# ZhentaoHuang/SealD-NeRF

Hardware: AMD Instinct MI355X
Metric: rendered rays/sec + sampled-points/sec, 800×800 D-NeRF jumpingjacks (higher is better)
Workload: dtype f16; 1 GPU; dnerf jumpingjacks-like 800x800 full-frame inference render, -O (fp16 field network, fp16 grid table), test sequence of 20 frames (camera orbit, one time stamp per frame, t = 0 .. 1: every frame selects its own occupancy slice, time encoding and the t == 0 canonical rule), T_thresh 1e-2, max_steps 1024, dt_gamma 0; rays=640000, field=fused, loop=device, frames_per_loop=4, rays_per_loop_on_this_gpu=2560000, frames_in_flight=4 loops of 4 frame(s) (the next starts when the newest is down to rays/2 alive), parallelism=single GPU

## Files before the change

### include/sdn_hip.h

```cpp
#ifndef SDN_HIP_H
#define SDN_HIP_H

#include <stdint.h>

#ifdef __cplusplus
extern "C" {
#endif

#define SDN_F32 0
#define SDN_F16 1

#define SDN_E_BADARG (-1)
#define SDN_E_UNSUPPORTED (-2)
#define SDN_E_TIMEOUT (-3)

const char *sdn_version(void);
int sdn_debug_shader_clock(unsigned long long *out4, uint32_t wall_ticks, void *stream);


int sdn_near_far_from_aabb(const float *rays_o, const float *rays_d, const float *aabb, uint32_t N,
                           float min_near, float *nears, float *fars, void *stream);

int sdn_sph_from_ray(const float *rays_o, const float *rays_d, float radius, uint32_t N, float *coords,
                     void *stream);
// ... 98 lines not shown

uint32_t sdn_field_basis_weight_floats_f32(void);
int sdn_field_basis_forward_f32(const float *xyzs, const float *dirs, const uint32_t *live_idx, const uint32_t *live_count,
                                uint32_t M, const float *weights, const float *basis_row , const float *table,
                                const int32_t *offsets_host, float S, uint32_t H, float bound, float density_scale,
                                float *sigmas, float *rgbs, void *stream);

uint32_t sdn_field_hyper_weight_blocks(void);
int sdn_field_hyper_forward_f16(const float *xyzs, const float *dirs, const uint32_t *live_idx, const uint32_t *live_count,
                                uint32_t M, const void *weights, const float *ambient_row , const void *table,
                                const int32_t *offsets_host, float S, uint32_t H, float bound, float density_scale,
                                float *sigmas, float *rgbs, void *stream);

void sdn_field_select_kernel(int persistent);
void sdn_field_persistent_workgroups(int n);

int sdn_field_build_quad_table(const void *embeddings, int dtype, const int32_t *ref_offsets_host, float S, uint32_t H, void *out,
                               void *stream);
int sdn_field_build_quad_table_nd(const void *embeddings, int dtype, uint32_t input_dim, const int32_t *ref_offsets_host, float S,
                                  uint32_t H, void *out, void *stream);

int sdn_density_query_cells_f16(const int32_t *cells, const uint32_t *cell_count, uint32_t n, const float *noise, uint32_t seed,
                                uint32_t grid_size, float cas_bound, const void *weights, const float *bias0, const void *table,
                                const int32_t *offsets_host, float S, uint32_t H, float bound, float density_scale, int zero_deform,
                                float *tmp_slice, void *stream);
int sdn_density_query_cells_f32(const int32_t *cells, const uint32_t *cell_count, uint32_t n, const float *noise, uint32_t seed,
                                uint32_t grid_size, float cas_bound, const float *weights, const float *bias0, const float *table,
                                const int32_t *offsets_host, float S, uint32_t H, float bound, float density_scale, int zero_deform,
                                float *tmp_slice, void *stream);
int sdn_density_query_cells_basis_f16(const int32_t *cells, const uint32_t *cell_count, uint32_t n, const float *noise, uint32_t seed,
// ... 110 lines not shown
    float *xyzs, *dirs, *deltas, *sigmas, *rgbs;
    uint32_t *live_idx;
    int32_t *live_counts, *state, *trace, *n_out;
    void *block_totals;
    const void *field_weights;
    const float *field_bias0;
    const void *grid_table;
    int32_t grid_offsets[17];
    float grid_S;
    uint32_t grid_H;
    uint32_t N, M_cap, n_counters, max_steps, C, H;
    float bound, dt_gamma, T_thresh, density_scale;
    int32_t zero_deform;
    const float *aabb;
    float min_near;
    int32_t reserved_;
    float *rays_tend;
    const struct SdnSealBox *seal;
    uint8_t *seal_mask;
    uint32_t n_group_frames, rays_per_frame;
    const uint8_t *frame_bitfield[SDN_MAX_GROUP_FRAMES];
    uint8_t *slot_frame;
    const void *frame_cull[SDN_MAX_GROUP_FRAMES];
    int32_t field_f32;
    int32_t reserved2_;
    const float *noises;
    const struct SdnSealBrush *seal_brush;
} SdnRenderCtx;

int sdn_render_begin(const SdnRenderCtx *ctx, void *stream);
int sdn_render_step_f16(const SdnRenderCtx *ctx, uint32_t bound_alive, void *stream);
int sdn_render_step_f16_ev(const SdnRenderCtx *ctx, uint32_t bound_alive, void *ev_field_begin, void *ev_field_end,
                           void *stream);
int sdn_render_time_kernel(int which);
int sdn_render_frame_f16(const SdnRenderCtx *ctx, float bg_color, float *image_out, float *depth_out, void *stream,
                         void *side_stream, void **ev_main, void **ev_copy, int32_t *host_snap, void **ev_field,
                         uint32_t max_field_events, uint32_t *iterations_out);
int sdn_render_frames_pipelined_f16(const SdnRenderCtx *const *ctxs, uint32_t n_ctx, uint32_t n_frames, const float *const *rays_o,
                                    const float *const *rays_d, float *const *image_outs, float *const *depth_outs, float bg_color,
                                    uint32_t overlap_div, void *const *streams, void *const *side_streams, void **ev_main,
// ... 133 lines not shown
```

### seald-nerf_amd/csrc/field.hip

```cpp
#include <math.h>
#include <type_traits>
#include <stdlib.h>

#include "sdn_common.h"
#include "sdn_internal.h"
#include "cell_points.h"
#include "grid_common.h"
#include "field_f16_net.h"

namespace {

using namespace sdn_f16;

#ifdef SDN_STAMPS
constexpr uint32_t kStampWGs = 2048;
__device__ unsigned long long g_field_stamps[kStampWGs * 2 * 32];
#define FSTAMP(k) do { __builtin_amdgcn_sched_barrier(0); if (stamp_on) { stamp_slot[k] = __builtin_amdgcn_s_memtime(); } __builtin_amdgcn_sched_barrier(0); } while (0)
#else
#define FSTAMP(k) ((void)0)
#endif

constexpr int kStageBytes = 32768;
constexpr int kWaves = 8;
constexpr int kPointsPerWG = 32 * kWaves;
// ... 270 lines not shown
    auto row = [&](uint32_t rr) {
        const T *p = emb + (size_t)(a + rr % hs) * 2;
        const __half2 v = __halves2half2(__float2half_rn((float)p[0]), __float2half_rn((float)p[1]));
        return __builtin_bit_cast(uint32_t, v);
    };
    out[i + 2u * l] = make_uint4(row(r), row(r + 1u), row(r + s1), row(r + s1 + 1u));
}

}

namespace sdn_int {

static int g_field_pp = -1;
static int g_field_pp_wgs = 0;
constexpr uint32_t kPPMinTilesPerCU = 4;

int field_table_layout(const int32_t *offsets_host) { return table_layout(offsets_host); }
int fill_tiled_levels_nd(TiledLevels &lv, uint32_t (*s3)[16], uint32_t D, const int32_t *offsets_host, float S, uint32_t H) {
    return fill_tiled_levels(lv, offsets_host, S, H, D, s3 ? *s3 : nullptr);
}
int fill_field_args(FieldArgs &a, TiledLevels &lv, const FieldCall &f) {
    int rc = fill_tiled_levels(lv, f.offsets_host, f.S, f.H);
    if (rc) return rc;
    fill_field_record(a, f);
    return 0;
}
void fill_field_record(FieldArgs &a, const FieldCall &f) {
    a.xyzs = f.xyzs; a.dirs = f.dirs; a.live_idx = f.live_idx; a.live_count = f.live_count; a.state = f.state; a.M = f.M;
    a.weights = (const unsigned char *)f.weights; a.bias0 = f.bias0; a.table = (const __half *)f.table;
    a.sigmas = f.sigmas; a.rgbs = f.rgbs; a.bound = f.bound; a.density_scale = f.density_scale; a.zero_deform = f.zero_deform;
// ... 28 lines not shown
    bool small = busy <= (uint32_t)cus;
    {
        static int pin = -1;
        if (pin < 0) {
            const char *e = getenv("SDN_FIELD_VARIANT");
            pin = !e ? 0 : (e[0] == 't' ? 1 : (e[0] == 'l' ? 2 : 0));
        }
        if (pin == 1) small = false;
        if (pin == 2) small = true;
    }
    const int layout = table_layout(f.offsets_host);
    if (g_field_pp < 0) {
        const char *e = getenv("SDN_FIELD_PP");
        g_field_pp = e ? atoi(e) : 1;
    }
    if (g_field_pp && layout == kLayoutQuad && busy >= kPPMinTilesPerCU * (uint32_t)cus && a.n_frames <= kPPMaxFrames && M < (1u << 28)) {
        const uint32_t pairs = sdn_div_up(M, kPPTile);
        int pp_cus = g_field_pp_wgs > 0 ? g_field_pp_wgs : cus;
        if (pp_cus > cus) pp_cus = cus;
        static int balance = -1;
        if (balance < 0) {
            const char *e = getenv("SDN_FIELD_PP_BALANCE");
            balance = e ? atoi(e) : 0;
        }
        const uint32_t grid = balance == 1 ? (uint32_t)cus : (uint32_t)pp_cus;
        a.pp_soft = (uint32_t)pp_cus | (balance == 0 ? 0x80000000u : (balance == 2 ? 0x40000000u : 0u));
        hipLaunchKernelGGL(k_field_pp_f16, dim3(pairs < grid ? pairs : grid), dim3(64 * kPPWaves), 0, st, a, lv);
        return sdn_launch_status();
    }
    launch_tile<false>(layout, small, wgs, a, lv, st);
    return sdn_launch_status();
}

int field_cells_f16(const FieldCells &q, hipStream_t st) {
    TiledLevels lv;
    FieldArgs a;
    int rc = fill_field_args(a, lv, q.f);
    if (rc) return rc;
    a.cell_noise = q.noise; a.cell_seed = q.seed;
    const float half_grid = q.cas_bound / (float)q.grid_size;
    a.cell_inv = 1.0f / (float)(q.grid_size - 1); a.cell_span = q.cas_bound - half_grid; a.cell_half = half_grid;
    const uint32_t wgs = sdn_div_up(q.f.M, (uint32_t)kPointsPerWG);
    const int layout = table_layout(q.f.offsets_host);
    if (layout == kLayoutRef) return SDN_E_UNSUPPORTED;
    launch_tile<true>(layout, wgs <= 256u, wgs, a, lv, st);
    return sdn_launch_status();
}

}

extern "C" {

uint32_t sdn_field_weight_blocks(void) { return (uint32_t)kBlkTotal; }

void sdn_field_select_kernel(int persistent) { sdn_int::g_field_pp = persistent; }
void sdn_field_persistent_workgroups(int n) { sdn_int::g_field_pp_wgs = n > 0 ? n : 0; }

int sdn_field_build_quad_table(const void *embeddings, int dtype, const int32_t *ref_offsets_host, float S, uint32_t H, void *out, void *stream) {
    return sdn_field_build_quad_table_nd(embeddings, dtype, 3, ref_offsets_host, S, H, out, stream);
}
int sdn_field_build_quad_table_nd(const void *embeddings, int dtype, uint32_t input_dim, const int32_t *ref_offsets_host, float S, uint32_t H, void *out,
                                  void *stream) {
    if (!embeddings || !ref_offsets_host || !out || ((uintptr_t)out & 15u) != 0) return SDN_E_BADARG;
    TiledLevels lv;
    uint32_t s3[16];
    int rc = fill_tiled_levels(lv, ref_offsets_host, S, H, input_dim, s3);
    if (rc) return rc;
    QuadLevels q;
    for (int l = 0; l < 17; l++) q.src[l] = (uint32_t)ref_offsets_host[l];
    for (int l = 0; l < 16; l++) q.s1[l] = lv.s1[l];
    const uint32_t rows = q.src[16];
// ... 19 lines not shown
}
uint32_t sdn_debug_field_stamp_words(void) { return kStampWGs * 2 * 32; }
int sdn_debug_field_stamps(unsigned long long *out) {
    if (!out) return SDN_E_BADARG;
    if (hipDeviceSynchronize() != hipSuccess) return sdn_launch_status();
    if (hipMemcpyFromSymbol(out, HIP_SYMBOL(g_field_stamps), sizeof(unsigned long long) * kStampWGs * 2 * 32) != hipSuccess) return sdn_launch_status();
    void *p = nullptr;
    if (hipGetSymbolAddress(&p, HIP_SYMBOL(g_field_stamps)) != hipSuccess) return sdn_launch_status();
    return (int)hipMemset(p, 0, sizeof(unsigned long long) * kStampWGs * 2 * 32);
}
#endif

int sdn_field_forward_f16(const float *xyzs, const float *dirs, const uint32_t *live_idx, const uint32_t *live_count, uint32_t M,
                          const void *weights, const float *bias0, const void *table, const int32_t *offsets_host, float S, uint32_t H,
                          float bound, float density_scale, int zero_deform, float *sigmas, float *rgbs, void *stream) {
    return sdn_int::field_forward_checked(0, {.xyzs = xyzs, .dirs = dirs, .live_idx = live_idx, .live_count = live_count, .M = M, .weights = weights,
                                              .bias0 = bias0, .table = table, .offsets_host = offsets_host, .S = S, .H = H, .bound = bound,
                                              .density_scale = density_scale, .zero_deform = zero_deform ? 1 : 0, .sigmas = sigmas, .rgbs = rgbs},
                                          stream);
}

}
```

### seald-nerf_amd/csrc/render.hip

```cpp
#include <atomic>
#include <chrono>
#include <stdio.h>
#include <stdlib.h>
#include <string.h>

#include "sdn_common.h"
#include "sdn_internal.h"

namespace sdn_int {
int render_begin(const SdnRenderCtx *c, void *mailbox, uint32_t frame_tag, hipStream_t st) {
    if (c->aabb) {
        int rc0 = sdn_near_far_from_aabb(c->rays_o, c->rays_d, c->aabb, c->N, c->min_near, (float *)c->nears, (float *)c->fars, st);
        if (rc0) return rc0;
    }
    int rc = loop_begin(*c, mailbox, frame_tag, st);
    if (rc) return rc;
    if (has_loop_cull(*c)) {
        const uint32_t nf = c->n_group_frames > 1 ? c->n_group_frames : 1u;
        bool kept = true;
        for (uint32_t f = 0; f < nf; f++) kept = kept && c->frame_cull[f] != nullptr;
        if (kept) rc = copy_cull(c->frame_cull, nf, (uint32_t *)c->cull_bits, st);
        else rc = c->n_group_frames > 1 ? build_cull_group(frame_sel(*c), (uint32_t *)c->cull_bits, st) : build_cull(c->bitfield, (uint32_t *)c->cull_bits, st);
        if (!rc && c->rays_tend) rc = loop_cull_start(*c, st);
    }
// ... 45 lines not shown
    int rc = 0;
    if (s->modify_hsv) rc = sdn_seal_modify_hsv(c.rgbs, c.seal_mask, m_slots, s->hsv[0], s->hsv[1], s->hsv[2], st);
    if (!rc && s->modify_rgb) {
        if (!s->scratch) return SDN_E_BADARG;
        rc = sdn_seal_modify_rgb(c.rgbs, c.seal_mask, m_slots, s->rgb[0], s->rgb[1], s->rgb[2], s->rgb_light_offset, s->scratch, c.live_idx,
                                 sdn_int::live_counters(c), c.state, st);
    }
    if (!rc && s->kind == SDN_SEAL_BRUSH && c.seal_brush && c.seal_brush->image) {
        if (!s->scratch) return SDN_E_BADARG;
        rc = sdn_seal_modify_image(c.rgbs, c.xyzs, c.seal_mask, m_slots, c.seal_brush->image, (char *)s->scratch + 32, c.live_idx,
                                   sdn_int::live_counters(c), c.state, st);
    }
    return rc;
}

static int launch_field(const SdnRenderCtx &c, uint32_t m_bound, uint32_t expect_points, hipStream_t st) {
    const bool group = c.n_group_frames > 1;
    return sdn_int::field_forward(c.field_f32,
                                  {.xyzs = c.xyzs, .dirs = c.dirs, .live_idx = c.live_idx, .live_count = sdn_int::live_counters(c), .state = c.state,
                                   .M = m_bound, .weights = c.field_weights, .bias0 = c.field_bias0, .table = c.grid_table,
                                   .offsets_host = c.grid_offsets, .S = c.grid_S, .H = c.grid_H, .bound = c.bound,
                                   .density_scale = c.density_scale, .zero_deform = c.zero_deform, .sigmas = c.sigmas, .rgbs = c.rgbs,
                                   .expect_points = expect_points, .slot_frame = group ? c.slot_frame : nullptr,
                                   .n_frames = group ? c.n_group_frames : 1u},
                                  st);
}

static uint32_t slot_bound(const SdnRenderCtx &c, uint32_t bound_alive) {
    const uint64_t m = (uint64_t)bound_alive * 8u;
    return m > c.N ? c.N : (uint32_t)m;
}
struct IterEvents { void *field0, *field1, *march0, *march1; };
static IterEvents split_events(void *e0, void *e1) {
    return g_timed_kernel.load() == 1 ? IterEvents{nullptr, nullptr, e0, e1} : IterEvents{e0, e1, nullptr, nullptr};
}
static void record(void *ev, hipStream_t st) { if (ev) (void)hipEventRecord((hipEvent_t)ev, st); }
static int map_field_color(const SdnRenderCtx &c, uint32_t m_slots, uint32_t expect_points, const IterEvents &ev, hipStream_t st) {
    int rc = seal_map(c, m_slots, st);
    if (rc) return rc;
    record(ev.field0, st);
    rc = launch_field(c, m_slots, expect_points, st);
    record(ev.field1, st);
    return rc ? rc : seal_color(c, m_slots, st);
}

static bool stepwise_noises_unsupported(const SdnRenderCtx *c) { return c->noises && c->n_group_frames > 1; }

static bool ctx_ok(const SdnRenderCtx *c) {
    if (!(c && c->rays_o && c->rays_d && c->nears && c->fars && c->alive_a && c->alive_b && c->rays_t && c->weights_sum &&
          c->depth && c->image && c->state && c->live_counts && c->cull_bits))
        return false;
    if (c->n_group_frames > 1) {
        if (c->n_group_frames > SDN_MAX_GROUP_FRAMES || !c->slot_frame || c->rays_per_frame == 0 ||
            (uint64_t)c->n_group_frames * c->rays_per_frame != c->N)
            return false;
        for (uint32_t f = 0; f < c->n_group_frames; f++)
// ... 1 lines not shown
        return true;
    }
    return c->bitfield != nullptr;
}

int sdn_render_begin(const SdnRenderCtx *c, void *stream) {
    if (!ctx_ok(c)) return SDN_E_BADARG;
    if (stepwise_noises_unsupported(c)) return SDN_E_UNSUPPORTED;
    return sdn_int::render_begin(c, nullptr, 0, (hipStream_t)stream);
}

int sdn_render_step_f16(const SdnRenderCtx *c, uint32_t bound_alive, void *stream) {
    return sdn_render_step_f16_ev(c, bound_alive, nullptr, nullptr, stream);
}

int sdn_render_step_f16_ev(const SdnRenderCtx *c, uint32_t bound_alive, void *ev_field_begin, void *ev_field_end, void *stream) {
    if (!c || bound_alive == 0) return SDN_E_BADARG;
    if (bound_alive > c->N) bound_alive = c->N;
    hipStream_t st = (hipStream_t)stream;
    const IterEvents ev = split_events(ev_field_begin, ev_field_end);
    record(ev.march0, st);
    int rc = sdn_int::loop_march(*c, bound_alive, st);
    record(ev.march1, st);
    if (!rc) rc = map_field_color(*c, slot_bound(*c, bound_alive), 0u, ev, st);
    return rc ? rc : sdn_int::loop_composite_compact(*c, bound_alive, st);
}

}

namespace {

constexpr uint32_t kRecompactMin = 8192;
uint32_t recompact_pct(uint32_t list_len) { return list_len > 81920u ? 95u : 50u; }
constexpr int kDriverTimeoutSeconds = 20;

struct FrameRun {
    const SdnRenderCtx *c;
    hipStream_t st, side;
    void **ev_main, **ev_copy, **ev_field;
    int32_t *host_snap;
    uint32_t max_field_events;
    uint32_t bound, it;
    bool steady, done;
    bool recompact = false;
    uint32_t list_bound = 0;
    void *mail_dev = nullptr;
    uint32_t tag = 0;
    uint32_t last_alive = 0;

    int begin() {
        if (!ctx_ok(c)) return SDN_E_BADARG;
        bound = c->N; it = 0; steady = false; done = false; last_alive = c->N; recompact = false; list_bound = 0;
        mail_dev = nullptr;
        unsigned int flags = 0;
        void *dptr = nullptr;
        if (hipHostGetFlags(&flags, host_snap) == hipSuccess && (flags & hipHostMallocCoherent) &&
            hipHostGetDevicePointer(&dptr, host_snap, 0) == hipSuccess && dptr) {
            static std::atomic<uint32_t> frame_seq{0};
            tag = (frame_seq.fetch_add(1) % 0x7FFFu) + 1u;
            mail_dev = dptr;
        } else {
            (void)hipGetLastError();
        }
        return sdn_int::render_begin(c, mail_dev, tag, st);
    }

    int enqueue() {
        void *e0 = (ev_field && it < max_field_events) ? ev_field[2 * it] : nullptr;
        void *e1 = (ev_field && it < max_field_events) ? ev_field[2 * it + 1] : nullptr;
        int rc;
        if (!steady) {
            rc = sdn_render_step_f16_ev(c, bound, e0, e1, st);
        } else {
            const IterEvents ev = split_events(e0, e1);
            rc = map_field_color(*c, slot_bound(*c, bound), last_alive * 8u, ev, st);
            if (!rc) record(ev.march0, st);
            if (!rc && recompact) {
                rc = sdn_int::loop_composite_compact(*c, bound, st, true);
                const uint32_t nb = last_alive < bound ? last_alive : bound;
                if (!rc) rc = sdn_int::loop_steady_begin(*c, nb, st, true);
                bound = list_bound = nb;
                recompact = false;
            } else if (!rc)
                rc = sdn_int::loop_composite_march(*c, bound, st);
            if (!rc) record(ev.march1, st);
        }
        if (rc) return rc;
        if (mail_dev) return 0;
        const uint32_t slot = it & 3u;
        hipError_t e = hipEventRecord((hipEvent_t)ev_main[slot], st);
// ... 108 lines not shown
        if (frame_times) {
            const SdnFrameTime &ft = frame_times[next];
            if (!ft.field_bias0 || !ft.bitfield[0]) return SDN_E_BADARG;
            local[slot].bitfield = ft.bitfield[0];
            for (uint32_t f = 0; f < SDN_MAX_GROUP_FRAMES; f++) local[slot].frame_bitfield[f] = ft.bitfield[f];
            for (uint32_t f = 0; f < SDN_MAX_GROUP_FRAMES; f++) local[slot].frame_cull[f] = ft.cull_grid[f];
            local[slot].field_bias0 = ft.field_bias0;
            local[slot].zero_deform = (int32_t)ft.zero_deform;
        }
        void **evf = ev_field_frames ? (void **)ev_field_frames[next] : nullptr;
        runs[slot] = FrameRun{&local[slot], (hipStream_t)streams[slot], (hipStream_t)side_streams[slot], ev_main + 4 * slot, ev_copy + 4 * slot,
                              evf, host_snap + 8 * slot, evf ? max_field_events : 0u, 0, 0, false, false};
        frame_of[slot] = (int)next++;
        return runs[slot].begin();
    };
    const bool stats = getenv("SDN_DRIVER_STATS") != nullptr;
    double t_work = 0, t_idle = 0;
    uint32_t n_loops = 0;
    auto now = [] { return std::chrono::duration<double, std::micro>(std::chrono::steady_clock::now().time_since_epoch()).count(); };
    auto launch_next = [&]() -> int {
        if (next >= n_frames) return 0;
        const uint32_t slot = next % n_ctx;
        if (frame_of[slot] >= 0) return 0;
        int newest = -1;
        bool any_active = false, excl_in_flight = false;
        for (uint32_t c = 0; c < n_ctx; c++) {
            if (frame_of[c] < 0) continue;
            any_active = true;
            if (newest < 0 || frame_of[c] > frame_of[newest]) newest = (int)c;
            if (exclusive_frames && exclusive_frames[frame_of[c]]) excl_in_flight = true;
        }
        bool ok = !any_active || (uint64_t)runs[newest].last_alive * overlap_div <= local[slot].N;
        if (exclusive_frames && any_active && (exclusive_frames[next] || excl_in_flight)) ok = false;
        if (!ok) return 0;
        int r = start(slot);
        if (!r) r = runs[slot].enqueue();
        return r;
    };
    auto fail = [&](int code) -> int {
        for (uint32_t c = 0; c < n_ctx; c++) { (void)hipStreamSynchronize((hipStream_t)streams[c]); (void)hipStreamSynchronize((hipStream_t)side_streams[c]); }
        (void)hipGetLastError();
        return code;
    };
    int rc = launch_next();
    if (rc) return fail(rc);
    auto t_last = stats ? now() : 0.0;
    uint32_t idle_spins = 0;
    auto t_progress = std::chrono::steady_clock::now();
    auto t_query = t_progress;
    while (finished < n_frames) {
        n_loops++;
// ... 9 lines not shown
            progress = true;
            rc = runs[s2].settle();
            if (rc) return fail(rc);
            if (runs[s2].done) {
                const int f = frame_of[s2];
                rc = sdn_render_finish(&local[s2], bg_color, image_outs[f], depth_outs[f], streams[s2]);
                if (rc) return fail(rc);
                if (done_events && done_events[f]) {
                    hipError_t e = hipEventRecord((hipEvent_t)done_events[f], (hipStream_t)streams[s2]);
                    if (e != hipSuccess) return fail((int)e);
                }
                if (iterations_out) __atomic_store_n(&iterations_out[f], runs[s2].it + 1, __ATOMIC_RELEASE);
                frame_of[s2] = -1;
                finished++;
            } else {
                rc = runs[s2].enqueue();
                if (rc) return fail(rc);
            }
            rc = launch_next();
            if (rc) return fail(rc);
        }
        if (!progress) {
            rc = launch_next();
            if (rc) return fail(rc);
            if ((++idle_spins & 0x3FFFu) == 0) {
                const auto now_c = std::chrono::steady_clock::now();
                if (now_c - t_progress > std::chrono::milliseconds(5) && now_c - t_query > std::chrono::milliseconds(5)) {
                    t_query = now_c;
                    for (uint32_t c = 0; c < n_ctx; c++)
                        if (frame_of[c] >= 0) { hipError_t q = hipStreamQuery((hipStream_t)streams[c]); if (q != hipSuccess && q != hipErrorNotReady) return fail((int)q); }
// ... 34 lines not shown
```

### seald-nerf_amd/csrc/sdn_internal.h

```cpp
#pragma once
#include "sdn_common.h"

namespace sdn_int {

struct FrameSel {
    uint32_t n_frames = 0;
    uint32_t rays_per_frame = 0;
    uint32_t cull_stride = 0;
    uint32_t pad_ = 0;
    const uint8_t *grid[SDN_MAX_GROUP_FRAMES] = {};
    uint8_t *slot_frame = nullptr;
};
FrameSel frame_sel(const SdnRenderCtx &c);

inline int32_t *snap_ring(const SdnRenderCtx &c) { return c.trace + 2 * (size_t)c.n_counters; }
inline int32_t *snap_n_out(const SdnRenderCtx &c) { return snap_ring(c) + 8; }
inline uint32_t *live_counters(const SdnRenderCtx &c) { return (uint32_t *)c.live_counts; }
inline float *jump_buffer(const SdnRenderCtx &c) { return c.rays_tend ? c.sigmas : nullptr; }
inline bool has_loop_cull(const SdnRenderCtx &c) { return c.H == 128 && c.C == 1; }
inline const uint32_t *loop_cull(const SdnRenderCtx &c) { return has_loop_cull(c) ? (const uint32_t *)c.cull_bits : nullptr; }

int loop_begin(const SdnRenderCtx &c, void *mailbox, uint32_t frame_tag, hipStream_t st);
int loop_cull_start(const SdnRenderCtx &c, hipStream_t st);
int loop_march(const SdnRenderCtx &c, uint32_t bound_alive, hipStream_t st);
// ... 15 lines not shown
    const int32_t *state = nullptr;
    uint32_t M = 0;
    const void *weights = nullptr;
    const float *bias0 = nullptr;
    const void *table = nullptr;
    const int32_t *offsets_host = nullptr;
    float S = 0;
    uint32_t H = 0;
    float bound = 0, density_scale = 0;
    int zero_deform = 0;
    float *sigmas = nullptr, *rgbs = nullptr;
    float *deform = nullptr;
    uint32_t expect_points = 0;
    const uint8_t *slot_frame = nullptr;
    uint32_t n_frames = 1;
};
struct FieldCells {
    FieldCall f;
    const float *noise = nullptr;
    uint32_t seed = 0, grid_size = 0;
    float cas_bound = 0;
};

inline uint32_t field_n_frames(const FieldCall &f) {
    if (!f.slot_frame || f.n_frames == 0) return 1u;
    return f.n_frames > (uint32_t)SDN_MAX_GROUP_FRAMES ? (uint32_t)SDN_MAX_GROUP_FRAMES : f.n_frames;
}

int field_forward_f16(const FieldCall &f, hipStream_t st);
int field_forward_f32(const FieldCall &f, hipStream_t st);
// ... 52 lines not shown
```

### seald-nerf_amd/dnerf_amd/frame_loops.py

```python
import ctypes
import os
import sys
from time import perf_counter
from types import SimpleNamespace

import numpy as np
import torch

import raymarching
import sdn_backend
from sdn_backend import lib, check, ptr, stream
from .dist import InOrderHandOn


def sample_capacity(N):
    return N + 128 + 8 * 128


def flat_rays(rays):
    return rays.contiguous().view(-1, 3)


def per_frame_times(time, n, mismatch, spread_single=False):
    times = list(time) if isinstance(time, (list, tuple)) else [time] * n
# ... 373 lines not shown
                raise RuntimeError(f"hipStreamCreateWithPriority failed ({rc})")
            out.append(torch.cuda.ExternalStream(h.value, device=device))
    _CONTEXT_STREAMS[key] = out
    return out


_CONTEXT_STREAMS = {}


class PipelinedDeviceLoop:

    def __init__(self, model, field, N, device, overlap_div=1, contexts=2, mailbox=True, **kw):
        self.N, self.device, self.overlap_div, self.K = N, device, int(overlap_div), int(contexts)
        self.loops = [DeviceLoop(model, field, N, device, mailbox=mailbox, **kw) for _ in range(self.K)]
        self.streams = _context_streams(self.K, device)
        if self.K > 1:
            lib.sdn_field_persistent_workgroups(int(torch.cuda.get_device_properties(device).multi_processor_count) * 7 // 8)
        self.host_state = sdn_backend.HostMailbox(self.K) if mailbox else torch.zeros(self.K, 8, dtype=torch.int32).pin_memory()
        self._ctxs = (ctypes.POINTER(sdn_backend.SdnRenderCtx) * self.K)(*[ctypes.pointer(lp.ctx) for lp in self.loops])
        self._fixed = None

    @torch.no_grad()
    def render_frames(self, rays_o, rays_d, time, bg_color=1.0, outputs=None, timing=None, exclusive=None, on_done=None, perturb=False,
                      noises=None):
        t_entry = perf_counter()
        if perturb or noises is not None:
            raise NotImplementedError("a perturbed first march is not built for pipelined frames: render preview frames with DeviceLoop")
        n = len(rays_o)
        assert n == len(rays_d) and n >= 1
        cur = torch.cuda.current_stream()
        ro = [flat_rays(r) for r in rays_o]
        rd = [flat_rays(r) for r in rays_d]
# ... 161 lines not shown
```

### seald-nerf_amd/sdn_backend.py

```python
import ctypes
import os
import weakref

import torch

_HERE = os.path.dirname(os.path.abspath(__file__))
LIB_PATH = os.environ.get("SDN_LIB_PATH") or os.path.join(_HERE, "lib", "libsdn_hip.so")

SDN_F32 = 0
SDN_F16 = 1

_c = ctypes
_vp, _u32, _f32, _i32, _u64 = _c.c_void_p, _c.c_uint32, _c.c_float, _c.c_int, _c.c_uint64

PROTOTYPES = {
    "sdn_near_far_from_aabb": [_vp, _vp, _vp, _u32, _f32, _vp, _vp, _vp],
    "sdn_sph_from_ray": [_vp, _vp, _f32, _u32, _vp, _vp],
    "sdn_get_rays": [_vp, _f32, _f32, _f32, _f32, _u32, _u32, _vp, _vp, _vp],
    "sdn_morton3D": [_vp, _u32, _vp, _vp],
    "sdn_morton3D_invert": [_vp, _u32, _vp, _vp],
    "sdn_packbits": [_vp, _u32, _f32, _vp, _vp],
    "sdn_march_rays_train": [_vp, _vp, _vp, _f32, _f32, _u32, _u32, _u32, _u32, _u32, _vp, _vp, _vp, _vp, _vp, _vp, _vp, _vp, _vp, _vp],
    "sdn_composite_rays_train_forward": [_vp, _vp, _vp, _vp, _u32, _u32, _f32, _vp, _vp, _vp, _vp],
    "sdn_composite_whole_rays": [_vp, _vp, _vp, _vp, _vp, _u32, _u32, _f32, _vp, _vp, _vp, _vp],
# ... 20 lines not shown
    "sdn_render_frame_f16": [_vp, _f32, _vp, _vp, _vp, _vp, _vp, _vp, _vp, _vp, _u32, _vp],
    "sdn_render_frames_pipelined_f16": [_vp, _u32, _u32, _vp, _vp, _vp, _vp, _f32, _u32, _vp, _vp, _vp, _vp, _vp, _vp, _u32, _vp, _vp, _vp, _vp],
    "sdn_host_mailbox_free": [_vp],
    "sdn_seal_bbox_map": [_vp, _vp, _u32, _vp, _u32, _vp, _u32, _vp, _vp, _vp, _vp, _vp, _vp, _vp],
    "sdn_seal_modify_hsv": [_vp, _vp, _u32, _f32, _f32, _f32, _vp],
    "sdn_seal_bbox_map_source": [_vp, _vp, _u32, _vp, _u32, _vp, _u32, _vp, _vp, _vp, _vp, _vp, _vp, _vp, _vp, _vp, _vp, _vp, _vp, _vp],
    "sdn_seal_anchor_map": [_vp, _vp, _u32, _vp, _u32, _vp, _u32, _vp, _vp, _vp, _vp, _f32, _f32, _vp, _vp, _vp, _vp, _vp, _vp, _vp],
    "sdn_seal_brush_map": [_vp, _vp, _u32, _vp, _u32, _vp, _u32, _vp, _vp, _vp, _f32, _u32, _vp, _u32, _vp, _vp],
    "sdn_seal_modify_rgb": [_vp, _vp, _u32, _f32, _f32, _f32, _f32, _vp, _vp, _vp, _vp, _vp],
    "sdn_whole_rays_schedule": [_vp, _vp, _vp, _u32, _u32, _f32, _u32, _vp, _vp, _vp, _vp],
    "sdn_seal_modify_rgb_whole_rays": [_vp, _vp, _vp, _vp, _vp, _u32, _u32, _f32, _u32, _f32, _f32, _f32, _f32, _vp, _vp, _vp, _vp, _vp],
    "sdn_seal_image_texels": [_vp, _u64, _vp],
    "sdn_seal_modify_image": [_vp, _vp, _vp, _u32, _vp, _vp, _vp, _vp, _vp, _vp],
    "sdn_seal_modify_image_whole_rays": [_vp, _vp, _vp, _vp, _vp, _vp, _u32, _u32, _f32, _u32, _vp, _vp, _vp, _vp, _vp, _vp],
    "sdn_field_forward_f16": [_vp, _vp, _vp, _vp, _u32, _vp, _vp, _vp, _vp, _f32, _u32, _f32, _f32, _i32, _vp, _vp, _vp],
    "sdn_field_forward_f32": [_vp, _vp, _vp, _vp, _u32, _vp, _vp, _vp, _vp, _f32, _u32, _f32, _f32, _i32, _vp, _vp, _vp, _vp],
    "sdn_field_forward_f32x3": [_vp, _vp, _vp, _vp, _u32, _vp, _vp, _vp, _vp, _f32, _u32, _f32, _f32, _i32, _vp, _vp, _vp, _vp],
    "sdn_field_basis_forward_f16": [_vp, _vp, _vp, _vp, _u32, _vp, _vp, _vp, _vp, _f32, _u32, _f32, _f32, _vp, _vp, _vp],
    "sdn_field_basis_forward_f32": [_vp, _vp, _vp, _vp, _u32, _vp, _vp, _vp, _vp, _f32, _u32, _f32, _f32, _vp, _vp, _vp],
    "sdn_density_query_cells_basis_f32": [_vp, _vp, _u32, _vp, _u32, _u32, _f32, _vp, _vp, _vp, _vp, _f32, _u32, _f32, _f32, _vp, _vp],
    "sdn_field_hyper_forward_f16": [_vp, _vp, _vp, _vp, _u32, _vp, _vp, _vp, _vp, _f32, _u32, _f32, _f32, _vp, _vp, _vp],
    "sdn_field_build_quad_table": [_vp, _i32, _vp, _f32, _u32, _vp, _vp],
    "sdn_field_build_quad_table_nd": [_vp, _i32, _u32, _vp, _f32, _u32, _vp, _vp],
    "sdn_grid_encode_forward_quad_f16": [_vp, _vp, _vp, _vp, _u32, _f32, _u32, _vp],
    "sdn_density_query_cells_f16": [_vp, _vp, _u32, _vp, _u32, _u32, _f32, _vp, _vp, _vp, _vp, _f32, _u32, _f32, _f32, _i32, _vp, _vp],
    "sdn_debug_shader_clock": [_vp, _u32, _vp],
    "sdn_density_query_cells_f32": [_vp, _vp, _u32, _vp, _u32, _u32, _f32, _vp, _vp, _vp, _vp, _f32, _u32, _f32, _f32, _i32, _vp, _vp],
    "sdn_density_query_cells_basis_f16": [_vp, _vp, _u32, _vp, _u32, _u32, _f32, _vp, _vp, _vp, _vp, _f32, _u32, _f32, _f32, _vp, _vp],
    "sdn_density_query_cells_hyper_f16": [_vp, _vp, _u32, _vp, _u32, _u32, _f32, _vp, _vp, _vp, _vp, _f32, _u32, _f32, _f32, _vp, _vp],
    "sdn_density_grid_ema": [_vp, _vp, ctypes.c_uint64, _f32, _vp, _vp],
# ... 9 lines not shown


class SdnFrameTime(ctypes.Structure):
    _fields_ = [("bitfield", _vp * MAX_GROUP_FRAMES), ("field_bias0", _vp), ("zero_deform", _u32), ("reserved_", _u32),
                ("cull_grid", _vp * MAX_GROUP_FRAMES)]


class SdnRenderCtx(ctypes.Structure):
    _fields_ = ([(n, _vp) for n in ("rays_o", "rays_d", "nears", "fars", "bitfield", "cull_bits", "alive_a", "alive_b", "rays_t",
                                   "weights_sum", "depth", "image", "xyzs", "dirs", "deltas", "sigmas", "rgbs", "live_idx",
                                   "live_counts", "state", "trace", "n_out", "block_totals", "field_weights", "field_bias0",
                                   "grid_table")]
                + [("grid_offsets", ctypes.c_int32 * 17), ("grid_S", _f32), ("grid_H", _u32)]
                + [(n, _u32) for n in ("N", "M_cap", "n_counters", "max_steps", "C", "H")]
                + [(n, _f32) for n in ("bound", "dt_gamma", "T_thresh", "density_scale")]
                + [("zero_deform", ctypes.c_int32), ("aabb", _vp), ("min_near", _f32), ("reserved_", ctypes.c_int32), ("rays_tend", _vp), ("seal", _vp), ("seal_mask", _vp),
                   ("n_group_frames", _u32), ("rays_per_frame", _u32), ("frame_bitfield", _vp * MAX_GROUP_FRAMES), ("slot_frame", _vp),
                   ("frame_cull", _vp * MAX_GROUP_FRAMES), ("field_f32", _i32), ("reserved2_", _i32), ("noises", _vp), ("seal_brush", _vp)])


LOOP_WORDS = ("n_alive", "n_step", "steps_done", "iteration", "side", "N", "max_steps", "advance_calls", "frozen_len", "survivors",
              "mailbox_lo", "mailbox_hi", "frame_tag", "tend_lo", "tend_hi", "culled_start")
(LOOP_N_ALIVE, LOOP_N_STEP, LOOP_STEPS_DONE, LOOP_ITERATION, LOOP_SIDE, LOOP_N, LOOP_MAX_STEPS, LOOP_ADVANCE_CALLS, LOOP_FROZEN_LEN,
 LOOP_SURVIVORS, LOOP_MAILBOX_LO, LOOP_MAILBOX_HI, LOOP_FRAME_TAG, LOOP_TEND_LO, LOOP_TEND_HI, LOOP_CULLED_START) = range(len(LOOP_WORDS))


class SdnSealBox(ctypes.Structure):
    _fields_ = [("bounds", _f32 * 24), ("n_bounds", _u32), ("n_tris", _u32), ("tris", _vp), ("test_dir", _f32 * 3), ("tinv", _f32 * 12),
                ("rinv", _f32 * 9), ("scale", _f32 * 3), ("center", _f32 * 3), ("hsv", _f32 * 3), ("modify_hsv", ctypes.c_int32),
                ("rgb", _f32 * 3), ("rgb_light_offset", _f32), ("modify_rgb", ctypes.c_int32), ("has_map_source", ctypes.c_int32),
                ("source_bound", _f32 * 6), ("map_source", _f32 * 3), ("reserved_", _u32), ("scratch", _vp), ("kind", _u32),
                ("v_anchor", _f32 * 3), ("v_offset", _f32 * 3), ("v_h", _f32 * 3), ("len_h", _f32), ("radius", _f32)]

# ... 265 lines not shown
```

Before: 3.220 billion sampled-points/s.

## Pick persistent field kernel workgroup share per loop from in-flight concurrency

Replaces the global 7/8-of-CUs persistent-workgroup cap, set once in Python when several contexts exist, with a per-loop share computed by the pipelined driver. A loop running alone with no loops waiting gets all CUs with balanced dealing. Otherwise it gets 7/8 of the CUs with exact dealing. The aim is to let tail loops use the whole GPU while keeping headroom for overlapping loops in steady state, at the cost of extra host logic per enqueue and possible contention changes.

```diff
diff --git a/include/sdn_hip.h b/include/sdn_hip.h
--- a/include/sdn_hip.h
+++ b/include/sdn_hip.h
@@ -136,6 +136,12 @@
 
 void sdn_field_select_kernel(int persistent);
 void sdn_field_persistent_workgroups(int n);
+int sdn_field_forward_f16_share(const float *xyzs, const float *dirs, const uint32_t *live_idx, const uint32_t *live_count,
+                                uint32_t M, const void *weights, const float *bias0, const void *table,
+                                const int32_t *offsets_host, float S, uint32_t H, float bound, float density_scale,
+                                int zero_deform, float *sigmas, float *rgbs, uint32_t pp_workgroups, uint32_t pp_deal,
+                                void *stream);
+int sdn_field_persistent_last_launch(uint32_t *out);
 
 int sdn_field_build_quad_table(const void *embeddings, int dtype, const int32_t *ref_offsets_host, float S, uint32_t H, void *out,
                                void *stream);
@@ -276,7 +282,7 @@
     int32_t zero_deform;
     const float *aabb;
     float min_near;
-    int32_t reserved_;
+    uint32_t pp_workgroups;
     float *rays_tend;
     const struct SdnSealBox *seal;
     uint8_t *seal_mask;
@@ -285,7 +291,7 @@
     uint8_t *slot_frame;
     const void *frame_cull[SDN_MAX_GROUP_FRAMES];
     int32_t field_f32;
-    int32_t reserved2_;
+    uint32_t pp_deal;
     const float *noises;
     const struct SdnSealBrush *seal_brush;
 } SdnRenderCtx;
diff --git a/seald-nerf_amd/csrc/field.hip b/seald-nerf_amd/csrc/field.hip
--- a/seald-nerf_amd/csrc/field.hip
+++ b/seald-nerf_amd/csrc/field.hip
@@ -1,4 +1,5 @@
 #include <math.h>
+#include <atomic>
 #include <type_traits>
 #include <stdlib.h>
 
@@ -308,6 +309,7 @@
 static int g_field_pp = -1;
 static int g_field_pp_wgs = 0;
 constexpr uint32_t kPPMinTilesPerCU = 4;
+static std::atomic<uint32_t> g_pp_launches{0}, g_pp_last_wgs{0}, g_pp_last_deal{0}, g_pp_last_grid{0};
 
 int field_table_layout(const int32_t *offsets_host) { return table_layout(offsets_host); }
 int fill_tiled_levels_nd(TiledLevels &lv, uint32_t (*s3)[16], uint32_t D, const int32_t *offsets_host, float S, uint32_t H) {
@@ -366,18 +368,22 @@
         const char *e = getenv("SDN_FIELD_PP");
         g_field_pp = e ? atoi(e) : 1;
     }
-    if (g_field_pp && layout == kLayoutQuad && busy >= kPPMinTilesPerCU * (uint32_t)cus && a.n_frames <= kPPMaxFrames && M < (1u << 28)) {
+    const uint32_t pp_min_tiles = g_field_pp > 1 ? (uint32_t)g_field_pp : kPPMinTilesPerCU * (uint32_t)cus;
+    if (g_field_pp && layout == kLayoutQuad && busy >= pp_min_tiles && a.n_frames <= kPPMaxFrames && M < (1u << 28)) {
         const uint32_t pairs = sdn_div_up(M, kPPTile);
-        int pp_cus = g_field_pp_wgs > 0 ? g_field_pp_wgs : cus;
-        if (pp_cus > cus) pp_cus = cus;
-        static int balance = -1;
-        if (balance < 0) {
+        const uint32_t pp_cus = f.pp_workgroups > 0 && f.pp_workgroups < (uint32_t)cus ? f.pp_workgroups : (uint32_t)cus;
+        static int balance_env = -2;
+        if (balance_env == -2) {
             const char *e = getenv("SDN_FIELD_PP_BALANCE");
-            balance = e ? atoi(e) : 0;
-        }
-        const uint32_t grid = balance == 1 ? (uint32_t)cus : (uint32_t)pp_cus;
-        a.pp_soft = (uint32_t)pp_cus | (balance == 0 ? 0x80000000u : (balance == 2 ? 0x40000000u : 0u));
-        hipLaunchKernelGGL(k_field_pp_f16, dim3(pairs < grid ? pairs : grid), dim3(64 * kPPWaves), 0, st, a, lv);
+            balance_env = e ? atoi(e) : -1;
+        }
+        const uint32_t balance = balance_env >= 0 ? (uint32_t)balance_env : f.pp_deal;
+        const uint32_t grid_cus = balance == kPPDealBalanced ? (uint32_t)cus : pp_cus;
+        const uint32_t grid = pairs < grid_cus ? pairs : grid_cus;
+        a.pp_soft = pp_cus | (balance == kPPDealExact ? 0x80000000u : (balance == kPPDealCapped ? 0x40000000u : 0u));
+        g_pp_last_wgs = pp_cus; g_pp_last_deal = balance; g_pp_last_grid = grid;
+        g_pp_launches++;
+        hipLaunchKernelGGL(k_field_pp_f16, dim3(grid), dim3(64 * kPPWaves), 0, st, a, lv);
         return sdn_launch_status();
     }
     launch_tile<false>(layout, small, wgs, a, lv, st);
@@ -407,6 +413,11 @@
 
 void sdn_field_select_kernel(int persistent) { sdn_int::g_field_pp = persistent; }
 void sdn_field_persistent_workgroups(int n) { sdn_int::g_field_pp_wgs = n > 0 ? n : 0; }
+int sdn_field_persistent_last_launch(uint32_t *out) {
+    if (!out) return SDN_E_BADARG;
+    out[0] = sdn_int::g_pp_launches; out[1] = sdn_int::g_pp_last_wgs; out[2] = sdn_int::g_pp_last_deal; out[3] = sdn_int::g_pp_last_grid;
+    return 0;
+}
 
 int sdn_field_build_quad_table(const void *embeddings, int dtype, const int32_t *ref_offsets_host, float S, uint32_t H, void *out, void *stream) {
     return sdn_field_build_quad_table_nd(embeddings, dtype, 3, ref_offsets_host, S, H, out, stream);
@@ -456,9 +467,18 @@
 int sdn_field_forward_f16(const float *xyzs, const float *dirs, const uint32_t *live_idx, const uint32_t *live_count, uint32_t M,
                           const void *weights, const float *bias0, const void *table, const int32_t *offsets_host, float S, uint32_t H,
                           float bound, float density_scale, int zero_deform, float *sigmas, float *rgbs, void *stream) {
+    return sdn_field_forward_f16_share(xyzs, dirs, live_idx, live_count, M, weights, bias0, table, offsets_host, S, H, bound, density_scale, zero_deform,
+                                       sigmas, rgbs, (uint32_t)sdn_int::g_field_pp_wgs, sdn_int::kPPDealExact, stream);
+}
+int sdn_field_forward_f16_share(const float *xyzs, const float *dirs, const uint32_t *live_idx, const uint32_t *live_count, uint32_t M,
+                                const void *weights, const float *bias0, const void *table, const int32_t *offsets_host, float S, uint32_t H,
+                                float bound, float density_scale, int zero_deform, float *sigmas, float *rgbs, uint32_t pp_workgroups,
+                                uint32_t pp_deal, void *stream) {
+    if (pp_deal > sdn_int::kPPDealCapped) return SDN_E_BADARG;
     return sdn_int::field_forward_checked(0, {.xyzs = xyzs, .dirs = dirs, .live_idx = live_idx, .live_count = live_count, .M = M, .weights = weights,
                                               .bias0 = bias0, .table = table, .offsets_host = offsets_host, .S = S, .H = H, .bound = bound,
-                                              .density_scale = density_scale, .zero_deform = zero_deform ? 1 : 0, .sigmas = sigmas, .rgbs = rgbs},
+                                              .density_scale = density_scale, .zero_deform = zero_deform ? 1 : 0, .sigmas = sigmas, .rgbs = rgbs,
+                                              .pp_workgroups = pp_workgroups, .pp_deal = pp_deal},
                                           stream);
 }
 
diff --git a/seald-nerf_amd/csrc/pp_share.h b/seald-nerf_amd/csrc/pp_share.h
--- /dev/null
+++ b/seald-nerf_amd/csrc/pp_share.h
@@ -0,0 +1,24 @@
+#pragma once
+#include <stdint.h>
+
+namespace sdn_int {
+
+enum : uint32_t {
+    kPPDealExact = 0,
+    kPPDealBalanced = 1,
+    kPPDealCapped = 2,
+};
+
+struct PPShare {
+    uint32_t workgroups;
+    uint32_t deal;
+};
+
+inline PPShare pp_share(uint32_t loops_in_flight, uint32_t loops_not_started, uint32_t cus) {
+    if (cus == 0) cus = 1;
+    if (loops_in_flight <= 1 && loops_not_started == 0) return {cus, kPPDealBalanced};
+    const uint32_t steady = cus * 7u / 8u;
+    return {steady ? steady : 1u, kPPDealExact};
+}
+
+}
diff --git a/seald-nerf_amd/csrc/render.hip b/seald-nerf_amd/csrc/render.hip
--- a/seald-nerf_amd/csrc/render.hip
+++ b/seald-nerf_amd/csrc/render.hip
@@ -83,7 +83,7 @@
     return rc;
 }
 
-static int launch_field(const SdnRenderCtx &c, uint32_t m_bound, uint32_t expect_points, hipStream_t st) {
+static int launch_field(const SdnRenderCtx &c, uint32_t m_bound, uint32_t expect_points, sdn_int::PPShare share, hipStream_t st) {
     const bool group = c.n_group_frames > 1;
     return sdn_int::field_forward(c.field_f32,
                                   {.xyzs = c.xyzs, .dirs = c.dirs, .live_idx = c.live_idx, .live_count = sdn_int::live_counters(c), .state = c.state,
@@ -91,8 +91,12 @@
                                    .offsets_host = c.grid_offsets, .S = c.grid_S, .H = c.grid_H, .bound = c.bound,
                                    .density_scale = c.density_scale, .zero_deform = c.zero_deform, .sigmas = c.sigmas, .rgbs = c.rgbs,
                                    .expect_points = expect_points, .slot_frame = group ? c.slot_frame : nullptr,
-                                   .n_frames = group ? c.n_group_frames : 1u},
+                                   .n_frames = group ? c.n_group_frames : 1u, .pp_workgroups = share.workgroups, .pp_deal = share.deal},
                                   st);
+}
+
+static sdn_int::PPShare ctx_share(const SdnRenderCtx &c) {
+    return c.pp_workgroups ? sdn_int::PPShare{c.pp_workgroups, c.pp_deal} : sdn_int::PPShare{0u, sdn_int::kPPDealExact};
 }
 
 static uint32_t slot_bound(const SdnRenderCtx &c, uint32_t bound_alive) {
@@ -104,11 +108,11 @@
     return g_timed_kernel.load() == 1 ? IterEvents{nullptr, nullptr, e0, e1} : IterEvents{e0, e1, nullptr, nullptr};
 }
 static void record(void *ev, hipStream_t st) { if (ev) (void)hipEventRecord((hipEvent_t)ev, st); }
-static int map_field_color(const SdnRenderCtx &c, uint32_t m_slots, uint32_t expect_points, const IterEvents &ev, hipStream_t st) {
+static int map_field_color(const SdnRenderCtx &c, uint32_t m_slots, uint32_t expect_points, sdn_int::PPShare share, const IterEvents &ev, hipStream_t st) {
     int rc = seal_map(c, m_slots, st);
     if (rc) return rc;
     record(ev.field0, st);
-    rc = launch_field(c, m_slots, expect_points, st);
+    rc = launch_field(c, m_slots, expect_points, share, st);
     record(ev.field1, st);
     return rc ? rc : seal_color(c, m_slots, st);
 }
@@ -140,16 +144,20 @@
     return sdn_render_step_f16_ev(c, bound_alive, nullptr, nullptr, stream);
 }
 
-int sdn_render_step_f16_ev(const SdnRenderCtx *c, uint32_t bound_alive, void *ev_field_begin, void *ev_field_end, void *stream) {
+static int step_ev(const SdnRenderCtx *c, uint32_t bound_alive, sdn_int::PPShare share, void *ev_field_begin, void *ev_field_end, hipStream_t st) {
     if (!c || bound_alive == 0) return SDN_E_BADARG;
     if (bound_alive > c->N) bound_alive = c->N;
-    hipStream_t st = (hipStream_t)stream;
     const IterEvents ev = split_events(ev_field_begin, ev_field_end);
     record(ev.march0, st);
     int rc = sdn_int::loop_march(*c, bound_alive, st);
     record(ev.march1, st);
-    if (!rc) rc = map_field_color(*c, slot_bound(*c, bound_alive), 0u, ev, st);
+    if (!rc) rc = map_field_color(*c, slot_bound(*c, bound_alive), 0u, share, ev, st);
     return rc ? rc : sdn_int::loop_composite_compact(*c, bound_alive, st);
+}
+
+int sdn_render_step_f16_ev(const SdnRenderCtx *c, uint32_t bound_alive, void *ev_field_begin, void *ev_field_end, void *stream) {
+    if (!c) return SDN_E_BADARG;
+    return step_ev(c, bound_alive, ctx_share(*c), ev_field_begin, ev_field_end, (hipStream_t)stream);
 }
 
 }
@@ -173,11 +181,13 @@
     void *mail_dev = nullptr;
     uint32_t tag = 0;
     uint32_t last_alive = 0;
+    sdn_int::PPShare share{0u, sdn_int::kPPDealExact};
 
     int begin() {
         if (!ctx_ok(c)) return SDN_E_BADARG;
         bound = c->N; it = 0; steady = false; done = false; last_alive = c->N; recompact = false; list_bound = 0;
         mail_dev = nullptr;
+        share = ctx_share(*c);
         unsigned int flags = 0;
         void *dptr = nullptr;
         if (hipHostGetFlags(&flags, host_snap) == hipSuccess && (flags & hipHostMallocCoherent) &&
@@ -196,10 +206,10 @@
         void *e1 = (ev_field && it < max_field_events) ? ev_field[2 * it + 1] : nullptr;
         int rc;
         if (!steady) {
-            rc = sdn_render_step_f16_ev(c, bound, e0, e1, st);
+            rc = step_ev(c, bound, share, e0, e1, st);
         } else {
             const IterEvents ev = split_events(e0, e1);
-            rc = map_field_color(*c, slot_bound(*c, bound), last_alive * 8u, ev, st);
+            rc = map_field_color(*c, slot_bound(*c, bound), last_alive * 8u, share, ev, st);
             if (!rc) record(ev.march0, st);
             if (!rc && recompact) {
                 rc = sdn_int::loop_composite_compact(*c, bound, st, true);
@@ -338,6 +348,34 @@
         frame_of[slot] = (int)next++;
         return runs[slot].begin();
     };
+    int cus = 0;
+    {
+        int dev = 0;
+        if (hipGetDevice(&dev) != hipSuccess || hipDeviceGetAttribute(&cus, hipDeviceAttributeMultiprocessorCount, dev) != hipSuccess || cus <= 0) {
+            (void)hipGetLastError();
+            cus = 256;
+        }
+    }
+    auto env_share = [](const char *name, sdn_int::PPShare &out) {
+        const char *e = getenv(name);
+        unsigned w = 0, d = 0;
+        if (!e || sscanf(e, "%u,%u", &w, &d) != 2 || d > sdn_int::kPPDealCapped) return false;
+        out = {w, d};
+        return true;
+    };
+    sdn_int::PPShare lone_env{}, steady_env{};
+    const bool has_lone_env = env_share("SDN_FIELD_PP_LONE", lone_env), has_steady_env = env_share("SDN_FIELD_PP_STEADY", steady_env);
+    auto set_share = [&](uint32_t slot) {
+        if (local[slot].pp_workgroups) return;
+        uint32_t in_flight = 0;
+        for (uint32_t c = 0; c < n_ctx; c++) in_flight += frame_of[c] >= 0 ? 1u : 0u;
+        const bool alone = exclusive_frames && exclusive_frames[frame_of[slot]];
+        const uint32_t flying = alone ? 1u : in_flight, waiting = (alone || n_ctx == 1) ? 0u : n_frames - next;
+        sdn_int::PPShare sh = sdn_int::pp_share(flying, waiting, (uint32_t)cus);
+        if (flying <= 1 && waiting == 0) { if (has_lone_env) sh = lone_env; }
+        else if (has_steady_env) sh = steady_env;
+        runs[slot].share = sh;
+    };
     const bool stats = getenv("SDN_DRIVER_STATS") != nullptr;
     double t_work = 0, t_idle = 0;
     uint32_t n_loops = 0;
@@ -358,7 +396,7 @@
         if (exclusive_frames && any_active && (exclusive_frames[next] || excl_in_flight)) ok = false;
         if (!ok) return 0;
         int r = start(slot);
-        if (!r) r = runs[slot].enqueue();
+        if (!r) { set_share(slot); r = runs[slot].enqueue(); }
         return r;
     };
     auto fail = [&](int code) -> int {
@@ -398,6 +436,7 @@
                 frame_of[s2] = -1;
                 finished++;
             } else {
+                set_share(s2);
                 rc = runs[s2].enqueue();
                 if (rc) return fail(rc);
             }
diff --git a/seald-nerf_amd/csrc/sdn_internal.h b/seald-nerf_amd/csrc/sdn_internal.h
--- a/seald-nerf_amd/csrc/sdn_internal.h
+++ b/seald-nerf_amd/csrc/sdn_internal.h
@@ -1,5 +1,6 @@
 #pragma once
 #include "sdn_common.h"
+#include "pp_share.h"
 
 namespace sdn_int {
 
@@ -53,6 +54,8 @@
     uint32_t expect_points = 0;
     const uint8_t *slot_frame = nullptr;
     uint32_t n_frames = 1;
+    uint32_t pp_workgroups = 0;
+    uint32_t pp_deal = 0;
 };
 struct FieldCells {
     FieldCall f;
diff --git a/seald-nerf_amd/dnerf_amd/frame_loops.py b/seald-nerf_amd/dnerf_amd/frame_loops.py
--- a/seald-nerf_amd/dnerf_amd/frame_loops.py
+++ b/seald-nerf_amd/dnerf_amd/frame_loops.py
@@ -411,8 +411,6 @@
         self.N, self.device, self.overlap_div, self.K = N, device, int(overlap_div), int(contexts)
         self.loops = [DeviceLoop(model, field, N, device, mailbox=mailbox, **kw) for _ in range(self.K)]
         self.streams = _context_streams(self.K, device)
-        if self.K > 1:
-            lib.sdn_field_persistent_workgroups(int(torch.cuda.get_device_properties(device).multi_processor_count) * 7 // 8)
         self.host_state = sdn_backend.HostMailbox(self.K) if mailbox else torch.zeros(self.K, 8, dtype=torch.int32).pin_memory()
         self._ctxs = (ctypes.POINTER(sdn_backend.SdnRenderCtx) * self.K)(*[ctypes.pointer(lp.ctx) for lp in self.loops])
         self._fixed = None
diff --git a/seald-nerf_amd/sdn_backend.py b/seald-nerf_amd/sdn_backend.py
--- a/seald-nerf_amd/sdn_backend.py
+++ b/seald-nerf_amd/sdn_backend.py
@@ -58,6 +58,8 @@
     "sdn_seal_modify_image": [_vp, _vp, _vp, _u32, _vp, _vp, _vp, _vp, _vp, _vp],
     "sdn_seal_modify_image_whole_rays": [_vp, _vp, _vp, _vp, _vp, _vp, _u32, _u32, _f32, _u32, _vp, _vp, _vp, _vp, _vp, _vp],
     "sdn_field_forward_f16": [_vp, _vp, _vp, _vp, _u32, _vp, _vp, _vp, _vp, _f32, _u32, _f32, _f32, _i32, _vp, _vp, _vp],
+    "sdn_field_forward_f16_share": [_vp, _vp, _vp, _vp, _u32, _vp, _vp, _vp, _vp, _f32, _u32, _f32, _f32, _i32, _vp, _vp, _u32, _u32, _vp],
+    "sdn_field_persistent_last_launch": [_vp],
     "sdn_field_forward_f32": [_vp, _vp, _vp, _vp, _u32, _vp, _vp, _vp, _vp, _f32, _u32, _f32, _f32, _i32, _vp, _vp, _vp, _vp],
     "sdn_field_forward_f32x3": [_vp, _vp, _vp, _vp, _u32, _vp, _vp, _vp, _vp, _f32, _u32, _f32, _f32, _i32, _vp, _vp, _vp, _vp],
     "sdn_field_basis_forward_f16": [_vp, _vp, _vp, _vp, _u32, _vp, _vp, _vp, _vp, _f32, _u32, _f32, _f32, _vp, _vp, _vp],
@@ -97,9 +99,9 @@
                 + [("grid_offsets", ctypes.c_int32 * 17), ("grid_S", _f32), ("grid_H", _u32)]
                 + [(n, _u32) for n in ("N", "M_cap", "n_counters", "max_steps", "C", "H")]
                 + [(n, _f32) for n in ("bound", "dt_gamma", "T_thresh", "density_scale")]
-                + [("zero_deform", ctypes.c_int32), ("aabb", _vp), ("min_near", _f32), ("reserved_", ctypes.c_int32), ("rays_tend", _vp), ("seal", _vp), ("seal_mask", _vp),
+                + [("zero_deform", ctypes.c_int32), ("aabb", _vp), ("min_near", _f32), ("pp_workgroups", _u32), ("rays_tend", _vp), ("seal", _vp), ("seal_mask", _vp),
                    ("n_group_frames", _u32), ("rays_per_frame", _u32), ("frame_bitfield", _vp * MAX_GROUP_FRAMES), ("slot_frame", _vp),
-                   ("frame_cull", _vp * MAX_GROUP_FRAMES), ("field_f32", _i32), ("reserved2_", _i32), ("noises", _vp), ("seal_brush", _vp)])
+                   ("frame_cull", _vp * MAX_GROUP_FRAMES), ("field_f32", _i32), ("pp_deal", _u32), ("noises", _vp), ("seal_brush", _vp)])
 
 
 LOOP_WORDS = ("n_alive", "n_step", "steps_done", "iteration", "side", "N", "max_steps", "advance_calls", "frozen_len", "survivors",
```

Measured after the change: 3.208 billion sampled-points/s. About the same (-0.4%).
